# jibanCat/gp_dla_detection

Measured on NVIDIA B200. Metric: qso_spectra_per_sec_10k_dla_samples, higher is better.
Workload: dtype f64

## Files before the change

### gp_dla_detection_b200/csrc/gpdla_i8_kernels.cuh

```cuda
#pragma once
#include "gpdla_kernels.cuh"

namespace gpdla {
namespace i8 {

constexpr int CLUSTER = 4;
constexpr int TS = 32;
constexpr int TM = CLUSTER * TS;
constexpr int WCTAS = 3;
constexpr int NPROD = 8;
constexpr int SPB = TS / NPROD;
constexpr int NCTRL = 4;
constexpr int THREADS = 32 * (NCTRL + NPROD);
constexpr int STAGES = 3;
constexpr double CAP = 0.996;
constexpr int TMEM_COLS = 512;
#ifndef GPDLA_I8P_PROBE
#define GPDLA_I8P_PROBE 0
#endif
constexpr int PROBE = GPDLA_I8P_PROBE;
#ifndef GPDLA_I8P_SHFL_CONV
#define GPDLA_I8P_SHFL_CONV 0
#endif
#ifndef GPDLA_I8P_PF
#define GPDLA_I8P_PF 0
#endif
#ifndef GPDLA_I8P_NCA
#define GPDLA_I8P_NCA 4
#endif
#ifndef GPDLA_I8P_PHASES
#define GPDLA_I8P_PHASES 0
#endif

template <int K, int L>
struct Shape {
  using G = GramShape<K>;
  static constexpr int WBLOCKS = (G::NPAIR <= WCTAS * 80) ? WCTAS : WCTAS + CLUSTER * ((G::NPAIR - WCTAS * 80 + CLUSTER * 80 - 1) / (CLUSTER * 80));
  static constexpr bool EXT = WBLOCKS > WCTAS;
  static constexpr int CPASSES = (WBLOCKS - WCTAS) / CLUSTER;
  static constexpr int NSLOT = WBLOCKS + 1;
  static constexpr int USLOT = WBLOCKS;
  static constexpr int WCOLS = (G::NPAIR + WBLOCKS - 1) / WBLOCKS;
  static constexpr int NW = (WCOLS + 15) / 16 * 16;
  static constexpr int NU = (K + 15) / 16 * 16;
  static constexpr int NMAX = NW > NU ? NW : NU;
  static constexpr int F = 8 * L - 1;
  static constexpr int LBO_A = 128;
  static constexpr int PLANE_A = (KC / 8) * LBO_A;
  static constexpr int SBO_A = PLANE_A * L;
  static constexpr int ROWBLOCK = (TS / 16) * SBO_A;
  static constexpr int A_TILE = (TM / 16) * SBO_A;
  static constexpr int BW_PLANE = NW * KC, BU_PLANE = NU * KC;
  static constexpr int L_BW = L * BW_PLANE;
  static constexpr int B_MAX = L * (BW_PLANE > BU_PLANE ? BW_PLANE : BU_PLANE);
  static constexpr int CHUNK_BYTES = L * (WBLOCKS * BW_PLANE + BU_PLANE);
  static constexpr int B_BUF = B_MAX;
  static constexpr int NCOLTAB = NSLOT * NMAX;
  static constexpr int CSTR = TS + 4;
  static constexpr int NENT = (K + 1) * (K + 2) / 2;
  static_assert(L * NW <= TMEM_COLS && L * NU <= TMEM_COLS, "diagonal accumulators must fit in TMEM");
  static_assert(WBLOCKS * WCOLS >= G::NPAIR && NW <= 80, "column blocks must cover the pair columns");
  static_assert(L >= 2 && L <= 7, "digit count");
  __host__ __device__ static constexpr int b_offset(int slot) { return slot * L * BW_PLANE; }
  __host__ __device__ static constexpr int b_bytes(int slot) { return L * (slot < WBLOCKS ? BW_PLANE : BU_PLANE); }
  __host__ __device__ static constexpr int slot_of_rank(int rank) { return rank < WCTAS ? rank : USLOT; }
  __host__ __device__ static constexpr int gram_column(int slot, int n) {
    return slot < WBLOCKS ? ((n < WCOLS && slot * WCOLS + n < G::NPAIR) ? slot * WCOLS + n : -1) : (n < K ? G::WT * 8 + n : -1);
  }
  __host__ __device__ static constexpr uint64_t digit_bias() {
    uint64_t b = 0;
    for (int i = 0; i < L; ++i) b |= (uint64_t)0x80 << (8 * i);
    return b;
  }
  __host__ __device__ static constexpr double magic() {
    double m = 1.5;
    for (int i = 0; i < 52 - F; ++i) m *= 2.0;
    return m;
  }
  static constexpr size_t OFF_A = 0;
  static constexpr size_t OFF_SX = OFF_A + (size_t)STAGES * A_TILE;
  static constexpr size_t OFF_B = OFF_SX + (size_t)STAGES * ROWBLOCK;
  static constexpr size_t OFF_CS = OFF_B + 2ull * B_BUF;
  static constexpr size_t OFF_RAW = OFF_CS + (EXT ? 0 : (size_t)NENT * CSTR * 8);
  static constexpr size_t OFF_MISC = OFF_RAW + (size_t)TS * RAWS * 8;
};

__constant__ short c_i8_stage[CLUSTER * 128];

struct I8Args {
  double* pix2;
  double* pix8;
  uint8_t* bop;
  double* colscale;
  double* colinv;
  int* status;
  int32_t* f64flag;
  int32_t* f64list;
  uint8_t* adig;
  unsigned long long* phase;
};

__device__ __forceinline__ unsigned long long* phase_ptr(const I8Args& xa) { return GPDLA_I8P_PHASES ? xa.phase : nullptr; }

__device__ __forceinline__ uint32_t cluster_ctarank() { uint32_t r; asm volatile("mov.u32 %0, %%cluster_ctarank;" : "=r"(r)); return r; }
__device__ __forceinline__ void cluster_sync_all() {
  asm volatile("barrier.cluster.arrive.release.aligned;" ::: "memory");
  asm volatile("barrier.cluster.wait.acquire.aligned;" ::: "memory");
}
__device__ __forceinline__ uint32_t mapa(uint32_t saddr, uint32_t rank) {
  uint32_t r;
  asm volatile("mapa.shared::cluster.u32 %0, %1, %2;" : "=r"(r) : "r"(saddr), "r"(rank));
  return r;
}
__device__ __forceinline__ void mbar_wait_d(uint64_t* bar, uint32_t parity, int* status, int code,
                                            unsigned long long* phase = nullptr, unsigned backoff_ns = 0) {
  const uint32_t a = smem_u32(bar);
  const long long t0 = phase ? clock64() : 0;
  for (uint32_t spins = 0;; ++spins) {
    uint32_t ok;
    asm volatile("{\n.reg .pred p;\nmbarrier.try_wait.parity.shared::cta.b64 p, [%1], %2;\nselp.u32 %0, 1, 0, p;\n}\n"
                 : "=r"(ok) : "r"(a), "r"(parity) : "memory");
    if (ok) break;
    if (backoff_ns) __nanosleep(backoff_ns);
    if (spins > 20000000u) {
      if (status) atomicExch(status, code + 100 * (int)(cluster_ctarank() + 1));
      __threadfence_system();
      asm volatile("trap;");
    }
  }
  if (phase) atomicAdd(&phase[8 + code], (unsigned long long)(clock64() - t0));
}
__device__ __forceinline__ void mbar_arrive_expect_tx(uint64_t* bar, uint32_t bytes) { mbar_expect_tx(bar, bytes); }
__device__ __forceinline__ void dsmem_bulk_copy(uint32_t dst_cluster, uint32_t src_cta, uint32_t bytes, uint32_t bar_cluster) {
  asm volatile("cp.async.bulk.shared::cluster.shared::cta.mbarrier::complete_tx::bytes [%0], [%1], %2, [%3];" ::"r"(dst_cluster),
               "r"(src_cta), "r"(bytes), "r"(bar_cluster)
               : "memory");
}
__device__ __forceinline__ void st_cluster_f64(uint32_t addr, double v) {
  asm volatile("st.shared::cluster.f64 [%0], %1;" ::"r"(addr), "d"(v) : "memory");
}
__device__ __forceinline__ uint64_t make_desc(uint32_t saddr, uint32_t lbo, uint32_t sbo) {
  return (uint64_t)((saddr >> 4) & 0x3FFF) | ((uint64_t)((lbo >> 4) & 0x3FFF) << 16) | ((uint64_t)((sbo >> 4) & 0x3FFF) << 32) |
         (1ull << 46);
}
__host__ __device__ constexpr uint32_t make_idesc(int n) {
  return (2u << 4) | (1u << 7) | (1u << 10) | (1u << 15) | ((uint32_t)(n >> 3) << 17) | ((uint32_t)(TM >> 4) << 24);
}
__device__ __forceinline__ void mma_i8(uint32_t tmem_d, uint64_t da, uint64_t db, uint32_t idesc, uint32_t accumulate) {
  asm volatile(
      "{\n.reg .pred p;\nsetp.ne.b32 p, %4, 0;\n"
      "tcgen05.mma.cta_group::1.kind::i8 [%0], %1, %2, %3, {%5, %5, %5, %5}, p;\n}\n" ::"r"(tmem_d),
      "l"(da), "l"(db), "r"(idesc), "r"(accumulate), "r"(0u)
      : "memory");
}
__device__ __forceinline__ void mma_commit(uint64_t* bar) {
  asm volatile("tcgen05.commit.cta_group::1.mbarrier::arrive::one.shared::cluster.b64 [%0];" ::"r"(smem_u32(bar)) : "memory");
}
__device__ __forceinline__ void mma_commit_multicast(uint64_t* bar, uint16_t mask) {
  asm volatile("tcgen05.commit.cta_group::1.mbarrier::arrive::one.shared::cluster.multicast::cluster.b64 [%0], %1;" ::"r"(
                   smem_u32(bar)),
               "h"(mask)
               : "memory");
}

__device__ __forceinline__ void bulk_store_global(void* dst, uint32_t src_cta, uint32_t bytes) {
  asm volatile("cp.async.bulk.global.shared::cta.bulk_group [%0], [%1], %2;" ::"l"(dst), "r"(src_cta), "r"(bytes) : "memory");
}
__device__ __forceinline__ void tma_load_1d_multicast(uint32_t dst_cta, const void* src, uint32_t bytes, uint32_t bar_cta, uint16_t mask) {
  asm volatile("cp.async.bulk.shared::cluster.global.mbarrier::complete_tx::bytes.multicast::cluster [%0], [%1], %2, [%3], %4;" ::"r"(dst_cta),
               "l"(src), "r"(bytes), "r"(bar_cta), "h"(mask)
               : "memory");
}

template <class Sh, int L, int N>
__device__ __forceinline__ void issue_chunk_mmas_fixed(uint32_t tmem_base, uint64_t da0, uint64_t db0, bool accumulate) {
  constexpr int group = 256 / N;
#pragma unroll
  for (int i = L - 1; i >= 0; --i) {
    const uint64_t da = da0 + (uint64_t)((i * Sh::PLANE_A) >> 4);
#pragma unroll
    for (int t0 = 0; t0 <= i; t0 += group) {
      const int nt = (PROBE & 32) ? 1 : ((group < i + 1 - t0) ? group : i + 1 - t0);
      const uint64_t db = db0 + (uint64_t)(((L - 1 - i + t0) * N * KC) >> 4);
      const uint32_t idesc = (PROBE & 16) ? (make_idesc(nt * N) & ~(0x1fu << 24)) | (4u << 24) : make_idesc(nt * N);
      mma_i8(tmem_base + (uint32_t)(t0 * N), da, db, idesc, (accumulate || i < L - 1) ? 1u : 0u);
    }
  }
}

template <int K, int L>
__global__ void __launch_bounds__(NTHREADS) i8_scales_kernel(const QuasarMeta* __restrict__ meta, const double* __restrict__ pix,
                                                             const double* __restrict__ Mq, const double* __restrict__ lam_pad,
                                                             const double* __restrict__ lamh, I8Args xa, int NPIX) {
  using Sh = Shape<K, L>;
  using G = GramShape<K>;
  const int q = blockIdx.x, tid = threadIdx.x;
  const double* pq = pix + (int64_t)q * NPIX * 4;
  double* p2 = xa.pix2 + (int64_t)q * NPIX * 2;
  double2* p8 = reinterpret_cast<double2*>(xa.pix8 + (int64_t)q * NPIX * 8);
  const double* lq = lam_pad + (int64_t)q * (NPIX + 8) + 6;
  const double* lhq = lamh + (int64_t)q * (NPIX + 8) + 6;
  bool unbounded = false;
  for (int i = tid; i < NPIX; i += NTHREADS) {
    const double y = pq[i * 4 + 0], v = pq[i * 4 + 1], mu = pq[i * 4 + 2], om2 = pq[i * 4 + 3];
    const double cw = CAP * (om2 + v);
    const double b = (v >= om2) ? 1.0 / (om2 + v) : 0.5 / sqrt(om2 * v);
    const double yy = fabs(y) + fabs(mu);
    unbounded |= !(v > 0.0) || !isfinite(b) || !isfinite(cw);
    const double cu = (yy > 0.0 && isfinite(b)) ? CAP / (b * yy) : 0.0;
    p2[i * 2 + 0] = cw; p2[i * 2 + 1] = cu;
    p8[i] = make_double2(lq[i], lhq[i]); p8[NPIX + i] = make_double2(y, v);
    p8[2 * NPIX + i] = make_double2(mu, om2); p8[3 * NPIX + i] = make_double2(cw, cu);
  }
  if (__syncthreads_or(unbounded) && tid == 0 && meta[q].nchunks > 0) {
    xa.f64flag[q] = 1;
    xa.f64list[1 + atomicAdd(&xa.f64list[0], 1)] = q;
  }
  const int n_u = meta[q].n_u;
  const double* mq = Mq + (int64_t)q * NPIX * K;
  __shared__ double sM[KC][K + 1];
// ... 213 lines not shown
    asm volatile("tcgen05.alloc.cta_group::1.sync.aligned.shared::cta.b32 [%0], %1;" ::"r"(smem_u32(s_tmem)), "n"(TMEM_COLS));
    asm volatile("tcgen05.relinquish_alloc_permit.cta_group::1.sync.aligned;");
  }
  asm volatile("tcgen05.fence::before_thread_sync;");
  __syncthreads();
  asm volatile("tcgen05.fence::after_thread_sync;");
  const uint32_t tmem_base = *s_tmem;
  cluster_sync_all();

  auto tile_live = [&](int q, const QuasarMeta& m) {
    return m.nchunks > 0 && !(args.active != nullptr && args.active[q] == 0) && xa.f64flag[q] == 0;
  };
  constexpr uint32_t b_bytes = (uint32_t)Sh::L_BW;
  if (warp == 0 && lane == 0) {
    const uint64_t da_stage0 = make_desc(smem_u32(At), Sh::LBO_A, Sh::SBO_A);
    const uint64_t db_buf0 = make_desc(smem_u32(Bt), 128, 256);
    int gc = 0, it = 0;
    for (int t = cluster_id; t < num_tiles; t += num_clusters) {
      const int q = (t % tiles_per_pass) / tiles_per_quasar;
      const QuasarMeta meta = args.meta[q];
      if (!tile_live(q, meta)) continue;
      if (it > 0) mbar_wait_d(bar_tfree, (it - 1) & 1, xa.status, 23, nullptr, 100);
      for (int c = 0; c < meta.nchunks; ++c, ++gc) {
        const int stage = gc % C_STAGES;
        mbar_wait_d(&bar_full[stage], (gc / C_STAGES) & 1, xa.status, 22, nullptr);
        asm volatile("tcgen05.fence::after_thread_sync;");
        const uint64_t da0 = da_stage0 + (uint64_t)(uint32_t)(stage * (Sh::A_TILE >> 4));
        const uint64_t db0 = db_buf0 + (uint64_t)(uint32_t)(stage * (Sh::L_BW >> 4));
        issue_chunk_mmas_fixed<Sh, L, Sh::NW>(tmem_base, da0, db0, c > 0);
        mma_commit_multicast(&bar_empty[stage], (uint16_t)((1u << CLUSTER) - 1));
      }
      mma_commit(bar_acc);
      ++it;
    }
  } else if (warp == 1 && lane == 0) {
    int gc = 0;
    for (int t = cluster_id; t < num_tiles; t += num_clusters) {
      const int pass = t / tiles_per_pass, qt = t % tiles_per_pass;
      const int q = qt / tiles_per_quasar;
      const QuasarMeta meta = args.meta[q];
      if (!tile_live(q, meta)) continue;
      const int slot = WCTAS + CLUSTER * pass + (int)rank;
      const uint8_t* asrc = xa.adig + (int64_t)qt * (args.NPIX / KC) * Sh::A_TILE + rank * Sh::ROWBLOCK;
      const uint8_t* bsrc = xa.bop + (int64_t)q * (args.NPIX / KC) * Sh::CHUNK_BYTES + Sh::b_offset(slot);
      for (int c = 0; c < meta.nchunks; ++c, ++gc) {
        const int stage = gc % C_STAGES;
        mbar_wait_d(&bar_empty[stage], ((gc / C_STAGES) & 1) ^ 1, xa.status, 21, nullptr, 50);
        mbar_expect_tx(&bar_full[stage], (uint32_t)Sh::A_TILE + b_bytes);
        tma_load_1d_multicast(smem_u32(At + stage * Sh::A_TILE) + rank * Sh::ROWBLOCK, asrc + (int64_t)c * Sh::A_TILE, Sh::ROWBLOCK,
                              smem_u32(&bar_full[stage]), (uint16_t)((1u << CLUSTER) - 1));
        tma_load_1d(Bt + stage * Sh::L_BW, bsrc + (int64_t)c * Sh::CHUNK_BYTES, b_bytes, &bar_full[stage]);
      }
    }
  } else if (warp >= 4) {
    const int e = warp & 3, half = (warp - 4) >> 2;
    constexpr int CHALF = (Sh::NW / 2 + 7) / 8 * 8;
    const uint32_t taddr0 = tmem_base + ((uint32_t)(e * 32) << 16);
    int it = 0;
    for (int t = cluster_id; t < num_tiles; t += num_clusters) {
      const int pass = t / tiles_per_pass, qt = t % tiles_per_pass;
      const int q = qt / tiles_per_quasar;
      const QuasarMeta meta = args.meta[q];
      if (!tile_live(q, meta)) continue;
      const int slot = WCTAS + CLUSTER * pass + (int)rank;
      if (lane == 0) mbar_wait_d(bar_acc, it & 1, xa.status, 24, nullptr, 200);
      __syncwarp();
      asm volatile("tcgen05.fence::after_thread_sync;");
      const int64_t row = (int64_t)(qt % tiles_per_quasar) * TM + e * 32 + lane;
      drain_to_gram<Sh, L>(taddr0, Sh::NW, slot, xa.colscale + (int64_t)q * Sh::NCOLTAB + slot * Sh::NMAX,
                           args.gram + ((int64_t)q * args.gram_rows + row) * Sh::G::NCOL, half * CHALF, (half + 1) * CHALF);
      asm volatile("tcgen05.fence::before_thread_sync;");
      __syncwarp();
      if (lane == 0) mbar_arrive(bar_tfree);
      ++it;
    }
  }
  __syncwarp();
  asm volatile("tcgen05.fence::before_thread_sync;");
  cluster_sync_all();
  asm volatile("tcgen05.fence::after_thread_sync;");
  if (warp == 0) asm volatile("tcgen05.dealloc.cta_group::1.sync.aligned.b32 %0, %1;" ::"r"(tmem_base), "n"(TMEM_COLS));
}

template <int K, int L>
struct PShape {
  using Sh = Shape<K, L>;
  static constexpr size_t OFF_MISC = Sh::OFF_MISC;
  __host__ __device__ static constexpr size_t smem_bytes(int num_lines) {
    return OFF_MISC + (size_t)TS * (num_lines + 6) * 8 + 128 * 8 + 4 * TS * 4 + 64 + (size_t)NPROD * 2 * SPB * KC * 8;
  }
};

template <int K, int L, int NL, int MODE>
__global__ void __cluster_dims__(CLUSTER, 1, 1) __launch_bounds__(P_THREADS, 1)
dla_loglik_i8p_kernel(LoglikArgs args, I8Args xa, int num_quasars, int tiles_per_quasar) {
  using Sh = Shape<K, L>;
  constexpr int CSTR = Sh::CSTR;
  const int tid = threadIdx.x, warp = tid >> 5, lane = tid & 31;
  const uint32_t rank = cluster_ctarank();
  const int64_t S = args.S;
  const int cluster_id = blockIdx.x / CLUSTER, num_clusters = gridDim.x / CLUSTER;
  const int num_tiles = num_quasars * tiles_per_quasar;

  extern __shared__ __align__(1024) unsigned char smem_raw[];
  uint8_t* At = smem_raw + Sh::OFF_A;
  uint8_t* Sx = smem_raw + Sh::OFF_SX;
  uint8_t* Bt = smem_raw + Sh::OFF_B;
  double* Cs = reinterpret_cast<double*>(smem_raw + Sh::OFF_CS);
  double* rawbuf = reinterpret_cast<double*>(smem_raw + Sh::OFF_RAW);
  double* s_nhi = reinterpret_cast<double*>(smem_raw + Sh::OFF_MISC);
  double* s_q = s_nhi + TS;
  double* s_ld = s_q + 2 * TS;
  double* s_mult = s_ld + 2 * TS;
  const int num_lines = (NL > 0) ? NL : args.num_lines;
  double* s_K = s_mult + (size_t)TS * num_lines;
  uint64_t* bars = reinterpret_cast<uint64_t*>(s_K + TS);
  uint64_t* bar_full = bars;
  uint64_t* bar_empty = bar_full + STAGES;
  uint64_t* bar_rows = bar_empty + STAGES;
  uint64_t* bar_pfull = bar_rows + STAGES;
  uint64_t* bar_pempty = bar_pfull + 2;
  uint64_t* bar_acc = bar_pempty + 2;
  uint64_t* bar_tfree = bar_acc + 1;
  uint64_t* bar_sq = bar_tfree + 1;
  uint64_t* bar_csfull = bar_sq + 2;
  uint64_t* bar_csfree = bar_csfull + 1;
  uint32_t* s_tmem = reinterpret_cast<uint32_t*>(bars + 32);
  uint64_t* bar_hfull = bars + 64;
  uint64_t* bar_hempty = bar_hfull + 2 * NPROD;
  int* s_part = reinterpret_cast<int*>(bars + 128);
  int* s_so = s_part + 3 * TS;
  double* hbuf = reinterpret_cast<double*>(s_so + TS + 16);

  if (tid == 0) {
    for (int i = 0; i < STAGES; ++i) { mbar_init(&bar_full[i], 1); mbar_init(&bar_empty[i], CLUSTER + (Sh::EXT ? 1 : 0)); mbar_init(&bar_rows[i], NPROD); }
    for (int i = 0; i < 2; ++i) { mbar_init(&bar_pfull[i], 1); mbar_init(&bar_pempty[i], 1); mbar_init(&bar_sq[i], NPROD); }
    mbar_init(bar_acc, 1); mbar_init(bar_tfree, 4); mbar_init(bar_csfull, CLUSTER);
    for (int i = 0; i < 2 * NPROD; ++i) { mbar_init(&bar_hfull[i], 1); mbar_init(&bar_hempty[i], 1); }
    for (int i = 0; i < CLUSTER; ++i) mbar_init(&bar_csfree[i], 4);
    asm volatile("fence.mbarrier_init.release.cluster;" ::: "memory");
  }
  if (warp == 0) {
    asm volatile("tcgen05.alloc.cta_group::1.sync.aligned.shared::cta.b32 [%0], %1;" ::"r"(smem_u32(s_tmem)), "n"(TMEM_COLS));
    asm volatile("tcgen05.relinquish_alloc_permit.cta_group::1.sync.aligned;");
  }
  asm volatile("tcgen05.fence::before_thread_sync;");
  __syncthreads();
  asm volatile("tcgen05.fence::after_thread_sync;");
  const uint32_t tmem_base = *s_tmem;
  cluster_sync_all();

  const int N = rank < WCTAS ? Sh::NW : Sh::NU;
  constexpr int NCA = (MODE == 0) ? GPDLA_I8P_NCA : SPB;
  constexpr bool CONV_B = NCA < SPB;
  constexpr bool SHFL_CONV = GPDLA_I8P_SHFL_CONV && !CONV_B && MODE != 2;
  const int slot = Sh::slot_of_rank((int)rank);
  const uint32_t b_bytes = (uint32_t)Sh::b_bytes(slot);
  auto tile_quasar = [&](int t) { return t / tiles_per_quasar; };
  auto tile_live = [&](int q, const QuasarMeta& m) {
    return m.nchunks > 0 && !(args.active != nullptr && args.active[q] == 0) && xa.f64flag[q] == 0;
  };

  if (warp >= NCTRL + 2 * NPROD) {
    asm volatile("setmaxnreg.inc.sync.aligned.u32 %0;" ::"n"(REG_EPI));
    const int e = warp - NCTRL - 2 * NPROD;
    const uint32_t cs_remote = mapa(smem_u32(Cs), (uint32_t)e) + (uint32_t)lane * 8;
    const uint32_t csfull_remote = mapa(smem_u32(bar_csfull), (uint32_t)e);
    const uint32_t taddr0 = tmem_base + ((uint32_t)(e * 32) << 16);
    int it = 0;
    for (int t = cluster_id; t < num_tiles; t += num_clusters) {
      const int q = tile_quasar(t);
      const QuasarMeta meta = args.meta[q];
      const int64_t s0 = (int64_t)(t % tiles_per_quasar) * TM + (int64_t)rank * TS;
      if (!tile_live(q, meta)) {
        if (lane < 8 && xa.f64flag[q] == 0) {
          const int64_t s = s0 + e * 8 + lane;
          if (s < S) args.sample_log_likelihoods[(int64_t)q * args.sll_stride + s] = NAN;
          else if (s == S && args.log_likelihoods_no_dla) args.log_likelihoods_no_dla[q] = NAN;
        }
        continue;
      }
      if (lane == 0) {
        mbar_wait_d(bar_acc, it & 1, xa.status, 6, phase_ptr(xa), 500);
        if (!Sh::EXT && it > 0) mbar_wait_cluster(&bar_csfree[e], (it - 1) & 1, xa.status, 10, phase_ptr(xa));
      }
      __syncwarp();
      asm volatile("tcgen05.fence::after_thread_sync;");
      const double* cs = xa.colscale + (int64_t)q * Sh::NCOLTAB + slot * Sh::NMAX;
      if constexpr (Sh::EXT) {
        drain_to_gram<Sh, L>(taddr0, N, slot, cs, args.gram + ((int64_t)q * args.gram_rows + (s0 - (int64_t)rank * TS) + e * 32 + lane) * Sh::G::NCOL);
        asm volatile("tcgen05.fence::before_thread_sync;");
        __syncwarp();
        if (lane == 0) mbar_arrive(bar_tfree);
        ++it;
        continue;
      }
      for (int c0 = 0; c0 < ((PROBE & 8) ? 0 : N); c0 += 8) {
        uint32_t v[L][8];
#pragma unroll
        for (int tt = 0; tt < L; ++tt) {
          asm volatile("tcgen05.ld.sync.aligned.32x32b.x8.b32 {%0,%1,%2,%3,%4,%5,%6,%7}, [%8];"
                       : "=r"(v[tt][0]), "=r"(v[tt][1]), "=r"(v[tt][2]), "=r"(v[tt][3]), "=r"(v[tt][4]), "=r"(v[tt][5]),
                         "=r"(v[tt][6]), "=r"(v[tt][7])
                       : "r"(taddr0 + (uint32_t)(tt * N + c0)));
        }
        asm volatile("tcgen05.wait::ld.sync.aligned;" ::: "memory");
#pragma unroll
        for (int jj = 0; jj < 8; ++jj) {
          const int idx = c_i8_stage[rank * 128 + c0 + jj];
          if (idx >= 0) {
            double acc = (double)(int32_t)v[L - 1][jj];
#pragma unroll
            for (int tt = L - 2; tt >= 0; --tt) acc = fma(acc, 256.0, (double)(int32_t)v[tt][jj]);
            st_cluster_f64(cs_remote + (uint32_t)(idx * CSTR * 8), acc * cs[c0 + jj]);
          }
        }
      }
      asm volatile("tcgen05.fence::before_thread_sync;");
      asm volatile("fence.acq_rel.cluster;" ::: "memory");
      __syncwarp();
      if (lane == 0) {
        mbar_arrive(bar_tfree);
        mbar_arrive_cluster(csfull_remote);
        mbar_wait_cluster(bar_csfull, it & 1, xa.status, 11, phase_ptr(xa));
        mbar_wait_d(&bar_sq[it & 1], (it >> 1) & 1, xa.status, 12, phase_ptr(xa), 200);
      }
      __syncwarp();
      if constexpr (!Sh::EXT) {
        if (!(PROBE & 8)) factor_staged<K, CSTR>(Cs, s_q + (it & 1) * TS, s_ld + (it & 1) * TS, e * 8, lane, meta, args, q, s0);
      }
      __syncwarp();
      if (lane == 0) {
        const uint32_t freebar = smem_u32(&bar_csfree[rank]);
        for (uint32_t peer = 0; peer < (uint32_t)CLUSTER; ++peer) mbar_arrive_cluster(mapa(freebar, peer));
      }
      ++it;
    }
  } else if (warp >= NCTRL + NPROD) {
    asm volatile("setmaxnreg.inc.sync.aligned.u32 %0;" ::"n"(REG_B));
    const int pr = warp - NCTRL - NPROD;
    const int row0 = pr * SPB;
    const uint32_t own_block = rank * Sh::ROWBLOCK;
    uint8_t* const wdst0 = (rank < WCTAS) ? At + own_block : Sx;
    uint8_t* const udst0 = (rank < WCTAS) ? Sx : At + own_block;
    const uint32_t wstride = (rank < WCTAS) ? Sh::A_TILE : Sh::ROWBLOCK;
    const uint32_t ustride = (rank < WCTAS) ? Sh::ROWBLOCK : Sh::A_TILE;
    const uint32_t rowoff = (row0 / 16) * Sh::SBO_A + (row0 % 16) + (lane / 8) * Sh::LBO_A + (lane % 8) * 16;
    constexpr uint64_t BIAS = Sh::digit_bias();
    const double MAGIC = Sh::magic();
    const uint64_t KADD = BIAS - (uint64_t)__double_as_longlong(MAGIC);
    const double* hb = hbuf + pr * (2 * SPB * KC) + lane;
    uint64_t* const hfull = bar_hfull + 2 * pr;
    uint64_t* const hempty = bar_hempty + 2 * pr;
    double* myraw = rawbuf + row0 * RAWS;
    int it = 0;
    int stage = 0;
    uint32_t empty_parity = 1;
    uint32_t gh = 0;
    long long w_empty = 0, w_hand = 0;
    for (int t = cluster_id; t < num_tiles; t += num_clusters) {
      const int q = tile_quasar(t);
      const QuasarMeta meta = args.meta[q];
      if (!tile_live(q, meta)) continue;
      const int64_t s0 = (int64_t)(t % tiles_per_quasar) * TM + (int64_t)rank * TS;
      const int nchunks = meta.nchunks;
      const double2* prec = reinterpret_cast<const double2*>(xa.pix8 + (int64_t)q * args.NPIX * 8) + lane;
      const int64_t PL = args.NPIX;
      double qacc[SPB], ldm[SPB];
      int lde[SPB];
#pragma unroll
      for (int ss = 0; ss < SPB; ++ss) { qacc[ss] = 0.0; ldm[ss] = 1.0; lde[ss] = 0; }
      double2 p01n = prec[PL], p23n = prec[2 * PL], p45n = prec[3 * PL];
      if (CONV_B) {
        const uint32_t slot = gh & 1u;
        mbar_wait_d(&hfull[slot], (gh >> 1) & 1u, xa.status, 14);
        if (lane < 6) {
#pragma unroll
          for (int ss = NCA; ss < SPB; ++ss) myraw[ss * RAWS + lane] = hb[(slot * SPB + ss) * KC];
        }
        __syncwarp();
        if (lane == 0) mbar_arrive(&hempty[slot]);
        ++gh;
      }
      for (int c = 0; c < nchunks; ++c) {
        const double y = p01n.x, v = p01n.y, mu = p23n.x, om2 = p23n.y, cw = p45n.x, cu = p45n.y;
        if (c + 1 < nchunks) {
          prec += KC;
          p01n = prec[PL]; p23n = prec[2 * PL]; p45n = prec[3 * PL];
        }
        const uint32_t slot = gh & 1u;
        long long tw0 = GPDLA_I8P_PHASES ? clock64() : 0;
        mbar_wait_d(&hfull[slot], (gh >> 1) & 1u, xa.status, 14);
        if (GPDLA_I8P_PHASES) w_hand += clock64() - tw0;
        double a[SPB];
#pragma unroll
        for (int ss = 0; ss < SPB; ++ss) a[ss] = hb[(slot * SPB + ss) * KC];
        __syncwarp();
        if (lane == 0) mbar_arrive(&hempty[slot]);
        ++gh;
        if (CONV_B) {
#pragma unroll
          for (int ss = NCA; ss < SPB; ++ss) myraw[ss * RAWS + 6 + lane] = a[ss];
          __syncwarp();
          double carry[SPB];
#pragma unroll
          for (int ss = NCA; ss < SPB; ++ss) {
            const double* rb = myraw + ss * RAWS;
            double acc_a = 0.0;
#pragma unroll
            for (int tt = 0; tt < 6; ++tt) acc_a = fma(rb[lane + tt], c_lines.ip[tt], acc_a);
            acc_a = fma(a[ss], c_lines.ip[6], acc_a);
            carry[ss] = rb[KC + (lane < 6 ? lane : 0)];
            a[ss] = (__double2hiint(a[ss]) < 0) ? 1.0 : acc_a;
          }
          __syncwarp();
          if (lane < 6) {
#pragma unroll
            for (int ss = NCA; ss < SPB; ++ss) myraw[ss * RAWS + lane] = carry[ss];
          }
        }
        uint64_t xw[SPB], xu[SPB];
#pragma unroll
        for (int ss = 0; ss < SPB; ++ss) {
          const double a2 = a[ss] * a[ss];
          const double d = fma(a2, om2, v);
          const double rd = fast_rcp(d);
          const double r = fma(-a[ss], mu, y);
          const double t1 = r * rd;
          xw[ss] = ((uint64_t)__double_as_longlong(fma(a2 * rd, cw, MAGIC)) + KADD) ^ BIAS;
          xu[ss] = ((uint64_t)__double_as_longlong(fma(a[ss] * t1, cu, MAGIC)) + KADD) ^ BIAS;
          qacc[ss] = fma(r, t1, qacc[ss]);
          ldm[ss] *= d;
        }
        tw0 = GPDLA_I8P_PHASES ? clock64() : 0;
        mbar_wait_d(&bar_empty[stage], empty_parity, xa.status, 1);
        if (GPDLA_I8P_PHASES) w_empty += clock64() - tw0;
        uint8_t* dW = wdst0 + stage * wstride + rowoff;
        uint8_t* dU = udst0 + stage * ustride + rowoff;
        if (PROBE & 4) {
          uint64_t sink = 0;
#pragma unroll
          for (int ss = 0; ss < SPB; ++ss) sink ^= xw[ss] ^ (xu[ss] << 1);
          if (sink == 0x123456789abcdefull) dW[0] = 1;
        } else {
          store_digit_planes<L, Sh::PLANE_A>(dW, xw);
          store_digit_planes<L, Sh::PLANE_A>(dU, xu);
          asm volatile("fence.proxy.async.shared::cta;" ::: "memory");
        }
        __syncwarp();
        if (lane == 0) mbar_arrive(&bar_rows[stage]);
        if (++stage == STAGES) { stage = 0; empty_parity ^= 1u; }
        if ((c & 7) == 7) {
#pragma unroll
          for (int ss = 0; ss < SPB; ++ss) {
            const int hi = __double2hiint(ldm[ss]);
            const int e2 = ((hi >> 20) & 0x7ff) - 1023;
            lde[ss] += e2;
            ldm[ss] = __hiloint2double(hi - (e2 << 20), __double2loint(ldm[ss]));
          }
        }
      }
#pragma unroll
      for (int ss = 0; ss < SPB; ++ss) {
        const double qs = warp_sum(qacc[ss]);
        const double ld = warp_sum(log(ldm[ss]) + (double)lde[ss] * 0.693147180559945309417);
        if (lane == 0) {
          if (Sh::EXT) {
            double* qd = args.qld + ((int64_t)q * args.gram_rows + s0 + row0 + ss) * 2;
            qd[0] = qs; qd[1] = ld;
          } else {
            s_q[(it & 1) * TS + row0 + ss] = qs; s_ld[(it & 1) * TS + row0 + ss] = ld;
          }
        }
      }
      __syncwarp();
      if (!Sh::EXT && lane == 0) mbar_arrive(&bar_sq[it & 1]);
      if (GPDLA_I8P_PHASES && xa.phase && lane == 0) {
        atomicAdd(&xa.phase[8 + 1], (unsigned long long)w_empty); atomicAdd(&xa.phase[8 + 14], (unsigned long long)w_hand);
        w_empty = w_hand = 0;
        if (pr == 0) atomicAdd(&xa.phase[7], 1ull);
      }
      ++it;
    }
  } else if (warp >= NCTRL) {
    asm volatile("setmaxnreg.inc.sync.aligned.u32 %0;" ::"n"(REG_A));
    const int pr = warp - NCTRL;
    const int row0 = pr * SPB;
    double* myraw = rawbuf + row0 * RAWS;
    double* hb = hbuf + pr * (2 * SPB * KC) + lane;
    uint64_t* const hfull = bar_hfull + 2 * pr;
    uint64_t* const hempty = bar_hempty + 2 * pr;
    uint32_t gh = 0;
    long long w_hand = 0;
    for (int t = cluster_id; t < num_tiles; t += num_clusters) {
      const int q = tile_quasar(t);
      const QuasarMeta meta = args.meta[q];
      if (!tile_live(q, meta)) continue;
      const int64_t s0 = (int64_t)(t % tiles_per_quasar) * TM + (int64_t)rank * TS;
      const int nchunks = meta.nchunks;
      __syncwarp();
      if (lane < SPB) {
        const int i = row0 + lane;
        const int64_t s = s0 + i;
        const bool is_null = s >= S;
        const int64_t so = sample_at(args, is_null ? S - 1 : s);
        const double z = __dadd_rn(meta.min_z_dla, __dmul_rn(meta.max_z_dla - meta.min_z_dla, args.offset_samples[so]));
        s_nhi[i] = is_null ? -1.0 : args.nhi_samples[so];
        s_K[i] = rest_table_offset(args.rt, z, meta.lam_ref);
        s_so[i] = (int)so;
        for (int j = 0; j < num_lines; ++j) s_mult[j * TS + i] = line_multiplier(j, z);
        if (MODE == 2) {
          for (int j = 0; j < args.num_partners; ++j)
            s_part[j * TS + i] = is_null ? 0 : args.partners[((int64_t)q * 3 + j) * S + so];
        }
      }
      __syncwarp();
      const double* lam = args.lam_pad + (int64_t)q * (args.NPIX + 8);
      const double2* pix8 = reinterpret_cast<const double2*>(xa.pix8 + (int64_t)q * args.NPIX * 8);
      double* const cache_q = (MODE != 0) ? args.acache + (int64_t)q * S * args.NPIX : nullptr;

      const double* lamh = args.lamh + (int64_t)q * (args.NPIX + 8);
      double K_mid;
      const int tab_mode = (MODE != 2) ? group_cell<SPB>(args.rt, s_K + row0, K_mid) : 0;
      auto eval_raw = [&](double lambda, double lh, double (&e)[SPB], const RestCell* cell = nullptr) {
        double tau[SPB];
        tau_samples<NL, SPB>(args.rt, tab_mode, K_mid, lambda, lh, s_mult + row0, TS, s_K + row0, num_lines, tau, cell);
        raw_from_tau<SPB, false>(tau, s_nhi + row0, e);
      };
      double eprev[SPB];
      if (MODE != 2) {
        double e[SPB];
        eval_raw(lam[lane < 6 ? lane : 5], lamh[lane < 6 ? lane : 5], e);
        if (CONV_B) {
          const uint32_t slot = gh & 1u;
          mbar_wait_d(&hempty[slot], ((gh >> 1) & 1u) ^ 1u, xa.status, 15);
#pragma unroll
          for (int ss = NCA; ss < SPB; ++ss) hb[(slot * SPB + ss) * KC] = e[ss];
          __syncwarp();
          if (lane == 0) mbar_arrive(&hfull[slot]);
          ++gh;
        }
        if (SHFL_CONV) {
#pragma unroll
          for (int ss = 0; ss < SPB; ++ss) eprev[ss] = __shfl_sync(0xffffffffu, e[ss], (lane + 6) & 31);
        } else if (lane < 6) {
#pragma unroll
          for (int ss = 0; ss < NCA; ++ss) myraw[ss * RAWS + lane] = e[ss];
        }
      }
      double rows_n[4][SPB];
      auto load_rows = [&](int ipix) {
#pragma unroll
        for (int ss = 0; ss < SPB; ++ss) rows_n[0][ss] = cache_q[(int64_t)s_so[row0 + ss] * args.NPIX + ipix];
#pragma unroll
        for (int j = 0; j < 3; ++j)
          if (j < args.num_partners) {
#pragma unroll
            for (int ss = 0; ss < SPB; ++ss) rows_n[1 + j][ss] = cache_q[(int64_t)s_part[j * TS + row0 + ss] * args.NPIX + ipix];
          }
      };
      if (MODE == 2) load_rows(lane);
      const double2* prec = pix8 + lane;
      double2 plln = prec[0];
      double2 plln2 = prec[nchunks > 1 ? KC : 0];
      RestCell cell_n;
      const bool use_cell = GPDLA_I8P_PF && MODE != 2 && tab_mode == 1;
      if (use_cell) rest_table_fetch(args.rt, plln.y, K_mid, cell_n);
      for (int c = 0; c < nchunks; ++c) {
        const int i = c * KC + lane;
        const double lambda = plln.x, lh = plln.y;
        const RestCell cell = cell_n;
        plln = plln2;
        if (c + 2 < nchunks) {
          prec += KC;
          plln2 = prec[KC];
        }
        if (use_cell && c + 1 < nchunks) rest_table_fetch(args.rt, plln.y, K_mid, cell_n);
        double a[SPB];
        if (MODE != 2) {
          double e[SPB];
          eval_raw(lambda, lh, e, use_cell ? &cell : nullptr);
          if (PROBE & 64) {
#pragma unroll
            for (int ss = 0; ss < SPB; ++ss) a[ss] = (__double2hiint(s_nhi[row0 + ss]) < 0) ? 1.0 : e[ss];
          } else {
#pragma unroll
            for (int ss = NCA; ss < SPB; ++ss) a[ss] = (__double2hiint(s_nhi[row0 + ss]) < 0) ? -1.0 : e[ss];
            if (SHFL_CONV) {
#pragma unroll
              for (int ss = 0; ss < SPB; ++ss) {
                double acc_a = 0.0;
#pragma unroll
                for (int tt = 0; tt < 6; ++tt) {
                  const int d = 6 - tt;
                  const double x = (lane >= 32 - d) ? eprev[ss] : e[ss];
                  acc_a = fma(__shfl_sync(0xffffffffu, x, (lane - d) & 31), c_lines.ip[tt], acc_a);
                }
                acc_a = fma(e[ss], c_lines.ip[6], acc_a);
                eprev[ss] = e[ss];
                a[ss] = (__double2hiint(s_nhi[row0 + ss]) < 0) ? 1.0 : acc_a;
              }
            } else if (NCA > 0) {
#pragma unroll
              for (int ss = 0; ss < NCA; ++ss) myraw[ss * RAWS + 6 + lane] = e[ss];
              __syncwarp();
              double carry[SPB];
#pragma unroll
              for (int ss = 0; ss < NCA; ++ss) {
                const double* rb = myraw + ss * RAWS;
                double acc_a = 0.0;
#pragma unroll
                for (int tt = 0; tt < 6; ++tt) acc_a = fma(rb[lane + tt], c_lines.ip[tt], acc_a);
                acc_a = fma(e[ss], c_lines.ip[6], acc_a);
                carry[ss] = rb[KC + (lane < 6 ? lane : 0)];
                a[ss] = (__double2hiint(s_nhi[row0 + ss]) < 0) ? 1.0 : acc_a;
              }
              __syncwarp();
              if (lane < 6) {
#pragma unroll
                for (int ss = 0; ss < NCA; ++ss) myraw[ss * RAWS + lane] = carry[ss];
              }
            }
          }
          if (MODE == 1) {
#pragma unroll
            for (int ss = 0; ss < SPB; ++ss)
              if (s0 + row0 + ss < S) cache_q[(int64_t)s_so[row0 + ss] * args.NPIX + i] = a[ss];
          }
        } else {
#pragma unroll
          for (int ss = 0; ss < SPB; ++ss) a[ss] = rows_n[0][ss];
#pragma unroll
          for (int j = 0; j < 3; ++j)
            if (j < args.num_partners) {
#pragma unroll
              for (int ss = 0; ss < SPB; ++ss) a[ss] = a[ss] * rows_n[1 + j][ss];
            }
          if (c + 1 < nchunks) load_rows(i + KC);
        }
        const uint32_t slot = gh & 1u;
        const long long tw0 = GPDLA_I8P_PHASES ? clock64() : 0;
        mbar_wait_d(&hempty[slot], ((gh >> 1) & 1u) ^ 1u, xa.status, 15);
        if (GPDLA_I8P_PHASES) w_hand += clock64() - tw0;
#pragma unroll
        for (int ss = 0; ss < SPB; ++ss) hb[(slot * SPB + ss) * KC] = a[ss];
        __syncwarp();
        if (lane == 0) mbar_arrive(&hfull[slot]);
        ++gh;
      }
      if (GPDLA_I8P_PHASES && xa.phase && lane == 0) { atomicAdd(&xa.phase[8 + 15], (unsigned long long)w_hand); w_hand = 0; }
    }
  } else {
    asm volatile("setmaxnreg.dec.sync.aligned.u32 %0;" ::"n"(REG_CTRL));
    if (warp == 0 && lane == 0) {
      static_assert(Sh::A_TILE % 16 == 0 && Sh::B_BUF % 16 == 0 && Sh::PLANE_A % 16 == 0, "descriptor offsets are in 16-byte units");
      const uint64_t da_stage0 = make_desc(smem_u32(At), Sh::LBO_A, Sh::SBO_A);
      const uint64_t db_buf0 = make_desc(smem_u32(Bt), 128, 256);
      int gc = 0, it = 0;
      for (int t = cluster_id; t < num_tiles; t += num_clusters) {
        const int q = tile_quasar(t);
        const QuasarMeta meta = args.meta[q];
        if (!tile_live(q, meta)) continue;
        const long long tile_t0 = GPDLA_I8P_PHASES ? clock64() : 0;
        if (it > 0) mbar_wait_d(bar_tfree, (it - 1) & 1, xa.status, 13, phase_ptr(xa), 100);
        for (int c = 0; c < meta.nchunks; ++c, ++gc) {
          const int stage = gc % STAGES, buf = gc & 1;
          mbar_wait_d(&bar_full[stage], (gc / STAGES) & 1, xa.status, 2, phase_ptr(xa), 100);
          mbar_wait_d(&bar_pfull[buf], (gc >> 1) & 1, xa.status, 3, phase_ptr(xa));
          asm volatile("tcgen05.fence::after_thread_sync;");
          const uint64_t da0 = da_stage0 + (uint64_t)(uint32_t)(stage * (Sh::A_TILE >> 4));
          const uint64_t db0 = db_buf0 + (uint64_t)(uint32_t)(buf * (Sh::B_BUF >> 4));
          if (PROBE & 1) { (void)da0; (void)db0; }
          else if (rank < WCTAS) issue_chunk_mmas_fixed<Sh, L, Sh::NW>(tmem_base, da0, db0, c > 0);
          else issue_chunk_mmas_fixed<Sh, L, Sh::NU>(tmem_base, da0, db0, c > 0);
          mma_commit_multicast(&bar_empty[stage], (uint16_t)((1u << CLUSTER) - 1));
          mma_commit(&bar_pempty[buf]);
        }
        mma_commit(bar_acc);
        if (GPDLA_I8P_PHASES && xa.phase) atomicAdd(&xa.phase[6], (unsigned long long)(clock64() - tile_t0));
        ++it;
      }
    } else if (warp == 1 && lane == 0) {
      int gc = 0;
      for (int t = cluster_id; t < num_tiles; t += num_clusters) {
        const int q = tile_quasar(t);
        const QuasarMeta meta = args.meta[q];
        if (!tile_live(q, meta)) continue;
        const uint8_t* bsrc = xa.bop + (int64_t)q * (args.NPIX / KC) * Sh::CHUNK_BYTES + Sh::b_offset(slot);
        for (int c = 0; c < meta.nchunks; ++c, ++gc) {
          const int buf = gc & 1;
          if (gc >= 2) mbar_wait_d(&bar_pempty[buf], ((gc >> 1) - 1) & 1, xa.status, 4, phase_ptr(xa), 100);
          mbar_expect_tx(&bar_pfull[buf], b_bytes);
          tma_load_1d(Bt + buf * Sh::B_BUF, bsrc + (int64_t)c * Sh::CHUNK_BYTES, b_bytes, &bar_pfull[buf]);
        }
      }
    } else if (warp == 2 && lane == 0) {
      int gc = 0;
      for (int t = cluster_id; t < num_tiles; t += num_clusters) {
        const int q = tile_quasar(t);
        const QuasarMeta meta = args.meta[q];
        if (!tile_live(q, meta)) continue;
        for (int c = 0; c < meta.nchunks; ++c, ++gc) {
          const int stage = gc % STAGES;
          mbar_wait_d(&bar_rows[stage], (gc / STAGES) & 1, xa.status, 5, phase_ptr(xa), 100);
          const uint32_t dst_off = smem_u32(At + stage * Sh::A_TILE) + rank * Sh::ROWBLOCK;
          const uint32_t other_rows = smem_u32(Sx + stage * Sh::ROWBLOCK);
          const uint32_t fullbar = smem_u32(&bar_full[stage]);
          if (PROBE & 2) { mbar_arrive(&bar_full[stage]); continue; }
          for (uint32_t peer = 0; peer < (uint32_t)CLUSTER; ++peer) {
            if (peer == rank) continue;
            const uint32_t src = (rank < WCTAS && peer < WCTAS) ? dst_off : other_rows;
            dsmem_bulk_copy(mapa(dst_off, peer), src, Sh::ROWBLOCK, mapa(fullbar, peer));
          }
          mbar_arrive_expect_tx(&bar_full[stage], (CLUSTER - 1) * Sh::ROWBLOCK);
          if constexpr (Sh::EXT) {
            uint8_t* gdst = xa.adig + (((int64_t)q * tiles_per_quasar + (t % tiles_per_quasar)) * (args.NPIX / KC) + c) * Sh::A_TILE +
                            rank * Sh::ROWBLOCK;
            bulk_store_global(gdst, (rank < WCTAS) ? dst_off : other_rows, Sh::ROWBLOCK);
            asm volatile("cp.async.bulk.commit_group;" ::: "memory");
            asm volatile("cp.async.bulk.wait_group.read 0;" ::: "memory");
            mbar_arrive(&bar_empty[stage]);
          }
        }
      }
    }
    __syncwarp();
  }
  asm volatile("tcgen05.fence::before_thread_sync;");
// ... 8 lines not shown
```

Before: 5704.

## Remap stage-B warps to sample-group by pixel-block tiles with shared hand-over slots

Stage-B consumer warps now cover 16 samples by 8 pixels each instead of 4 samples by 32 pixels. Hand-over buffers are shared per group of four warps, with an XOR-swizzled layout and 2 or 3 slots depending on the line count. The per-sample reductions become a cross-warp named-barrier tree plus shuffles. The split-convolution path (NCA) is removed, so the producers always do the full convolution. The goal is bank-conflict-free digit stores into the MMA tile, checked by constexpr asserts. The cost is extra named-barrier syncs in the reduction and coupling between warps through group-level mbarriers.

```diff
diff --git a/gp_dla_detection_b200/csrc/gpdla_i8_kernels.cuh b/gp_dla_detection_b200/csrc/gpdla_i8_kernels.cuh
--- a/gp_dla_detection_b200/csrc/gpdla_i8_kernels.cuh
+++ b/gp_dla_detection_b200/csrc/gpdla_i8_kernels.cuh
@@ -24,9 +24,6 @@
 #endif
 #ifndef GPDLA_I8P_PF
 #define GPDLA_I8P_PF 0
-#endif
-#ifndef GPDLA_I8P_NCA
-#define GPDLA_I8P_NCA 4
 #endif
 #ifndef GPDLA_I8P_PHASES
 #define GPDLA_I8P_PHASES 0
@@ -136,6 +133,10 @@
                "r"(src_cta), "r"(bytes), "r"(bar_cluster)
                : "memory");
 }
+template <int ID, int THREADS>
+__device__ __forceinline__ void named_barrier_sync() {
+  asm volatile("bar.sync %0, %1;" ::"n"(ID), "n"(THREADS) : "memory");
+}
 __device__ __forceinline__ void st_cluster_f64(uint32_t addr, double v) {
   asm volatile("st.shared::cluster.f64 [%0], %1;" ::"r"(addr), "d"(v) : "memory");
 }
@@ -515,12 +516,114 @@
   if (warp == 0) asm volatile("tcgen05.dealloc.cta_group::1.sync.aligned.b32 %0, %1;" ::"r"(tmem_base), "n"(TMEM_COLS));
 }
 
+struct StageB {
+  static constexpr int GROUPS = TS / 16;
+  static constexpr int WARPS = NPROD / GROUPS;
+  static constexpr int HAND_SLOT = 16 * KC;
+  __host__ __device__ static constexpr int hand_slots(int num_lines) { return num_lines <= 3 ? 3 : 2; }
+  static constexpr int RED = GROUPS * 2 * SPB * 32;
+  __host__ __device__ static constexpr int group(int pr) { return pr / WARPS; }
+  __host__ __device__ static constexpr int pblock(int pr) { return pr % WARPS; }
+  __host__ __device__ static constexpr int sample(int pr, int lane, int ss) { return 16 * group(pr) + SPB * (lane & 3) + ss; }
+  __host__ __device__ static constexpr int pixel(int pr, int lane) { return 8 * pblock(pr) + (lane >> 2); }
+  __host__ __device__ static constexpr int hand(int sl, int pix) { return sl * KC + (pix ^ (8 * ((sl / SPB) & 1))); }
+  template <class Sh>
+  __host__ __device__ static constexpr int tile_byte(int sample, int pix) {
+    return (sample / 16) * Sh::SBO_A + (pix / 8) * Sh::LBO_A + (pix % 8) * 16 + sample % 16;
+  }
+};
+
+__host__ __device__ constexpr int bank_wavefronts(const int (&addr)[32], int bytes) {
+  int words[32][64] = {}, n[32] = {}, worst = 0;
+  for (int l = 0; l < 32; ++l)
+    for (int w = addr[l] / 4; w < (addr[l] + bytes) / 4; ++w) {
+      bool seen = false;
+      for (int i = 0; i < n[w % 32]; ++i) seen |= words[w % 32][i] == w;
+      if (!seen) words[w % 32][n[w % 32]++] = w;
+      worst = n[w % 32] > worst ? n[w % 32] : worst;
+    }
+  return worst;
+}
+template <class Sh>
+__host__ __device__ constexpr bool stage_b_stores_conflict_free() {
+  for (int pr = 0; pr < NPROD; ++pr) {
+    int addr[32] = {};
+    for (int l = 0; l < 32; ++l) {
+      addr[l] = StageB::tile_byte<Sh>(StageB::sample(pr, l, 0), StageB::pixel(pr, l));
+      if (addr[l] % 4 != 0) return false;
+    }
+    if (bank_wavefronts(addr, 4) != 1) return false;
+  }
+  return Sh::PLANE_A % 128 == 0 && Sh::SBO_A % 128 == 0;
+}
+__host__ __device__ constexpr int hand_over_wavefronts(bool b_read) {
+  int worst = 0;
+  for (int pr = 0; pr < NPROD; ++pr)
+    for (int ss = 0; ss < SPB; ++ss) {
+      int addr[32] = {};
+      for (int l = 0; l < 32; ++l)
+        addr[l] = 8 * (b_read ? StageB::hand(StageB::sample(pr, l, ss) % 16, StageB::pixel(pr, l)) : StageB::hand((pr * SPB + ss) % 16, l));
+      const int w = bank_wavefronts(addr, 8);
+      worst = w > worst ? w : worst;
+    }
+  return worst;
+}
+__host__ __device__ constexpr bool stage_b_tiles_block() {
+  unsigned cover[TS] = {};
+  for (int pr = 0; pr < NPROD; ++pr)
+    for (int l = 0; l < 32; ++l)
+      for (int ss = 0; ss < SPB; ++ss) {
+        const int s = StageB::sample(pr, l, ss), p = StageB::pixel(pr, l);
+        if (s < 0 || s >= TS || p < 0 || p >= KC || ((cover[s] >> p) & 1u)) return false;
+        cover[s] |= 1u << p;
+        if (StageB::group(pr) != s / 16 || StageB::hand(s % 16, p) != StageB::hand(s % 16 - ss, p) + ss * KC) return false;
+      }
+  for (int s = 0; s < TS; ++s)
+    if (cover[s] != 0xffffffffu) return false;
+  return true;
+}
+static_assert(KC == 32 && TS == 32 && SPB == 4 && StageB::WARPS * 8 == KC, "stage-B mapping: 2 groups x 4 pixel blocks of 8");
+static_assert(stage_b_tiles_block(), "stage-B warps must tile the chunk's (sample, pixel) block exactly");
+static_assert(hand_over_wavefronts(true) == 2 && hand_over_wavefronts(false) == 2, "hand-over accesses: 2 wavefronts per 256 bytes");
+
+__device__ __forceinline__ void group_sum(double (&v)[SPB], double* red, int g, int pb) {
+  auto sync = [g] {
+    if (g == 0) named_barrier_sync<1, 32 * StageB::WARPS>();
+    else named_barrier_sync<2, 32 * StageB::WARPS>();
+  };
+  static_assert(StageB::GROUPS == 2, "one named barrier per group");
+  if (pb >= 2) {
+#pragma unroll
+    for (int ss = 0; ss < SPB; ++ss) red[((pb & 1) * SPB + ss) * 32] = v[ss];
+  }
+  sync();
+  if (pb < 2) {
+#pragma unroll
+    for (int ss = 0; ss < SPB; ++ss) v[ss] += red[((pb & 1) * SPB + ss) * 32];
+  }
+  if (pb == 1) {
+#pragma unroll
+    for (int ss = 0; ss < SPB; ++ss) red[(SPB + ss) * 32] = v[ss];
+  }
+  sync();
+  if (pb == 0) {
+#pragma unroll
+    for (int ss = 0; ss < SPB; ++ss) {
+      v[ss] += red[(SPB + ss) * 32];
+#pragma unroll
+      for (int o = 16; o >= 4; o >>= 1) v[ss] += __shfl_xor_sync(0xffffffffu, v[ss], o);
+    }
+  }
+  sync();
+}
+
 template <int K, int L>
 struct PShape {
   using Sh = Shape<K, L>;
   static constexpr size_t OFF_MISC = Sh::OFF_MISC;
   __host__ __device__ static constexpr size_t smem_bytes(int num_lines) {
-    return OFF_MISC + (size_t)TS * (num_lines + 6) * 8 + 128 * 8 + 4 * TS * 4 + 64 + (size_t)NPROD * 2 * SPB * KC * 8;
+    return OFF_MISC + (size_t)TS * (num_lines + 6) * 8 + 128 * 8 + 4 * TS * 4 + 64 + (size_t)StageB::GROUPS * StageB::hand_slots(num_lines) * StageB::HAND_SLOT * 8 +
+           (size_t)StageB::RED * 8;
   }
 };
 
@@ -559,17 +662,23 @@
   uint64_t* bar_csfull = bar_sq + 2;
   uint64_t* bar_csfree = bar_csfull + 1;
   uint32_t* s_tmem = reinterpret_cast<uint32_t*>(bars + 32);
+  constexpr int HS = (NL > 0) ? StageB::hand_slots(NL) : 2;
   uint64_t* bar_hfull = bars + 64;
-  uint64_t* bar_hempty = bar_hfull + 2 * NPROD;
+  uint64_t* bar_hempty = bar_hfull + HS * StageB::GROUPS;
   int* s_part = reinterpret_cast<int*>(bars + 128);
   int* s_so = s_part + 3 * TS;
   double* hbuf = reinterpret_cast<double*>(s_so + TS + 16);
+  double* s_red = hbuf + StageB::GROUPS * HS * StageB::HAND_SLOT;
+  static_assert(stage_b_stores_conflict_free<Sh>(), "stage-B digit stores must be one wavefront each");
+  static_assert(PShape<K, L>::smem_bytes(MAX_LINES) <= 227 * 1024 && PShape<K, L>::smem_bytes(3) <= 227 * 1024,
+                "shared memory beyond the opt-in limit");
+  static_assert(2 * HS * StageB::GROUPS <= 64, "hand-over barriers must fit their 64 slots");
 
   if (tid == 0) {
     for (int i = 0; i < STAGES; ++i) { mbar_init(&bar_full[i], 1); mbar_init(&bar_empty[i], CLUSTER + (Sh::EXT ? 1 : 0)); mbar_init(&bar_rows[i], NPROD); }
     for (int i = 0; i < 2; ++i) { mbar_init(&bar_pfull[i], 1); mbar_init(&bar_pempty[i], 1); mbar_init(&bar_sq[i], NPROD); }
     mbar_init(bar_acc, 1); mbar_init(bar_tfree, 4); mbar_init(bar_csfull, CLUSTER);
-    for (int i = 0; i < 2 * NPROD; ++i) { mbar_init(&bar_hfull[i], 1); mbar_init(&bar_hempty[i], 1); }
+    for (int i = 0; i < HS * StageB::GROUPS; ++i) { mbar_init(&bar_hfull[i], StageB::WARPS); mbar_init(&bar_hempty[i], StageB::WARPS); }
     for (int i = 0; i < CLUSTER; ++i) mbar_init(&bar_csfree[i], 4);
     asm volatile("fence.mbarrier_init.release.cluster;" ::: "memory");
   }
@@ -584,9 +693,7 @@
   cluster_sync_all();
 
   const int N = rank < WCTAS ? Sh::NW : Sh::NU;
-  constexpr int NCA = (MODE == 0) ? GPDLA_I8P_NCA : SPB;
-  constexpr bool CONV_B = NCA < SPB;
-  constexpr bool SHFL_CONV = GPDLA_I8P_SHFL_CONV && !CONV_B && MODE != 2;
+  constexpr bool SHFL_CONV = GPDLA_I8P_SHFL_CONV && MODE != 2;
   const int slot = Sh::slot_of_rank((int)rank);
   const uint32_t b_bytes = (uint32_t)Sh::b_bytes(slot);
   auto tile_quasar = [&](int t) { return t / tiles_per_quasar; };
@@ -672,20 +779,20 @@
   } else if (warp >= NCTRL + NPROD) {
     asm volatile("setmaxnreg.inc.sync.aligned.u32 %0;" ::"n"(REG_B));
     const int pr = warp - NCTRL - NPROD;
-    const int row0 = pr * SPB;
+    const int g = StageB::group(pr), pb = StageB::pblock(pr);
+    const int pix = StageB::pixel(pr, lane);
     const uint32_t own_block = rank * Sh::ROWBLOCK;
-    uint8_t* const wdst0 = (rank < WCTAS) ? At + own_block : Sx;
-    uint8_t* const udst0 = (rank < WCTAS) ? Sx : At + own_block;
+    const uint32_t rowoff = StageB::tile_byte<Sh>(StageB::sample(pr, lane, 0), pix);
+    uint8_t* const wdst0 = ((rank < WCTAS) ? At + own_block : Sx) + rowoff;
+    uint8_t* const udst0 = ((rank < WCTAS) ? Sx : At + own_block) + rowoff;
     const uint32_t wstride = (rank < WCTAS) ? Sh::A_TILE : Sh::ROWBLOCK;
     const uint32_t ustride = (rank < WCTAS) ? Sh::ROWBLOCK : Sh::A_TILE;
-    const uint32_t rowoff = (row0 / 16) * Sh::SBO_A + (row0 % 16) + (lane / 8) * Sh::LBO_A + (lane % 8) * 16;
     constexpr uint64_t BIAS = Sh::digit_bias();
     const double MAGIC = Sh::magic();
     const uint64_t KADD = BIAS - (uint64_t)__double_as_longlong(MAGIC);
-    const double* hb = hbuf + pr * (2 * SPB * KC) + lane;
-    uint64_t* const hfull = bar_hfull + 2 * pr;
-    uint64_t* const hempty = bar_hempty + 2 * pr;
-    double* myraw = rawbuf + row0 * RAWS;
+    const double* hb = hbuf + g * (HS * StageB::HAND_SLOT) + StageB::hand(StageB::sample(pr, lane, 0) % 16, pix);
+    uint64_t* const hfull = bar_hfull + HS * g;
+    uint64_t* const hempty = bar_hempty + HS * g;
     int it = 0;
     int stage = 0;
     uint32_t empty_parity = 1;
@@ -697,61 +804,29 @@
       if (!tile_live(q, meta)) continue;
       const int64_t s0 = (int64_t)(t % tiles_per_quasar) * TM + (int64_t)rank * TS;
       const int nchunks = meta.nchunks;
-      const double2* prec = reinterpret_cast<const double2*>(xa.pix8 + (int64_t)q * args.NPIX * 8) + lane;
+      const double2* prec = reinterpret_cast<const double2*>(xa.pix8 + (int64_t)q * args.NPIX * 8) + pix;
       const int64_t PL = args.NPIX;
       double qacc[SPB], ldm[SPB];
       int lde[SPB];
 #pragma unroll
       for (int ss = 0; ss < SPB; ++ss) { qacc[ss] = 0.0; ldm[ss] = 1.0; lde[ss] = 0; }
       double2 p01n = prec[PL], p23n = prec[2 * PL], p45n = prec[3 * PL];
-      if (CONV_B) {
-        const uint32_t slot = gh & 1u;
-        mbar_wait_d(&hfull[slot], (gh >> 1) & 1u, xa.status, 14);
-        if (lane < 6) {
-#pragma unroll
-          for (int ss = NCA; ss < SPB; ++ss) myraw[ss * RAWS + lane] = hb[(slot * SPB + ss) * KC];
-        }
-        __syncwarp();
-        if (lane == 0) mbar_arrive(&hempty[slot]);
-        ++gh;
-      }
       for (int c = 0; c < nchunks; ++c) {
         const double y = p01n.x, v = p01n.y, mu = p23n.x, om2 = p23n.y, cw = p45n.x, cu = p45n.y;
         if (c + 1 < nchunks) {
           prec += KC;
           p01n = prec[PL]; p23n = prec[2 * PL]; p45n = prec[3 * PL];
         }
-        const uint32_t slot = gh & 1u;
+        const uint32_t slot = gh % HS;
         long long tw0 = GPDLA_I8P_PHASES ? clock64() : 0;
-        mbar_wait_d(&hfull[slot], (gh >> 1) & 1u, xa.status, 14);
+        mbar_wait_d(&hfull[slot], (gh / HS) & 1u, xa.status, 14);
         if (GPDLA_I8P_PHASES) w_hand += clock64() - tw0;
         double a[SPB];
 #pragma unroll
-        for (int ss = 0; ss < SPB; ++ss) a[ss] = hb[(slot * SPB + ss) * KC];
+        for (int ss = 0; ss < SPB; ++ss) a[ss] = hb[slot * StageB::HAND_SLOT + ss * KC];
         __syncwarp();
         if (lane == 0) mbar_arrive(&hempty[slot]);
         ++gh;
-        if (CONV_B) {
-#pragma unroll
-          for (int ss = NCA; ss < SPB; ++ss) myraw[ss * RAWS + 6 + lane] = a[ss];
-          __syncwarp();
-          double carry[SPB];
-#pragma unroll
-          for (int ss = NCA; ss < SPB; ++ss) {
-            const double* rb = myraw + ss * RAWS;
-            double acc_a = 0.0;
-#pragma unroll
-            for (int tt = 0; tt < 6; ++tt) acc_a = fma(rb[lane + tt], c_lines.ip[tt], acc_a);
-            acc_a = fma(a[ss], c_lines.ip[6], acc_a);
-            carry[ss] = rb[KC + (lane < 6 ? lane : 0)];
-            a[ss] = (__double2hiint(a[ss]) < 0) ? 1.0 : acc_a;
-          }
-          __syncwarp();
-          if (lane < 6) {
-#pragma unroll
-            for (int ss = NCA; ss < SPB; ++ss) myraw[ss * RAWS + lane] = carry[ss];
-          }
-        }
         uint64_t xw[SPB], xu[SPB];
 #pragma unroll
         for (int ss = 0; ss < SPB; ++ss) {
@@ -768,8 +843,8 @@
         tw0 = GPDLA_I8P_PHASES ? clock64() : 0;
         mbar_wait_d(&bar_empty[stage], empty_parity, xa.status, 1);
         if (GPDLA_I8P_PHASES) w_empty += clock64() - tw0;
-        uint8_t* dW = wdst0 + stage * wstride + rowoff;
-        uint8_t* dU = udst0 + stage * ustride + rowoff;
+        uint8_t* dW = wdst0 + stage * wstride;
+        uint8_t* dU = udst0 + stage * ustride;
         if (PROBE & 4) {
           uint64_t sink = 0;
 #pragma unroll
@@ -793,16 +868,20 @@
           }
         }
       }
-#pragma unroll
-      for (int ss = 0; ss < SPB; ++ss) {
-        const double qs = warp_sum(qacc[ss]);
-        const double ld = warp_sum(log(ldm[ss]) + (double)lde[ss] * 0.693147180559945309417);
-        if (lane == 0) {
+      double* const red = s_red + g * (2 * SPB * 32) + lane;
+      group_sum(qacc, red, g, pb);
+#pragma unroll
+      for (int ss = 0; ss < SPB; ++ss) ldm[ss] = log(ldm[ss]) + (double)lde[ss] * 0.693147180559945309417;
+      group_sum(ldm, red, g, pb);
+      if (pb == 0 && lane < 4) {
+        const int row0 = 16 * g + SPB * lane;
+#pragma unroll
+        for (int ss = 0; ss < SPB; ++ss) {
           if (Sh::EXT) {
             double* qd = args.qld + ((int64_t)q * args.gram_rows + s0 + row0 + ss) * 2;
-            qd[0] = qs; qd[1] = ld;
+            qd[0] = qacc[ss]; qd[1] = ldm[ss];
           } else {
-            s_q[(it & 1) * TS + row0 + ss] = qs; s_ld[(it & 1) * TS + row0 + ss] = ld;
+            s_q[(it & 1) * TS + row0 + ss] = qacc[ss]; s_ld[(it & 1) * TS + row0 + ss] = ldm[ss];
           }
         }
       }
@@ -820,9 +899,10 @@
     const int pr = warp - NCTRL;
     const int row0 = pr * SPB;
     double* myraw = rawbuf + row0 * RAWS;
-    double* hb = hbuf + pr * (2 * SPB * KC) + lane;
-    uint64_t* const hfull = bar_hfull + 2 * pr;
-    uint64_t* const hempty = bar_hempty + 2 * pr;
+    const int g = StageB::group(pr);
+    double* hb = hbuf + g * (HS * StageB::HAND_SLOT) + StageB::hand(row0 % 16, lane);
+    uint64_t* const hfull = bar_hfull + HS * g;
+    uint64_t* const hempty = bar_hempty + HS * g;
     uint32_t gh = 0;
     long long w_hand = 0;
     for (int t = cluster_id; t < num_tiles; t += num_clusters) {
@@ -864,21 +944,12 @@
       if (MODE != 2) {
         double e[SPB];
         eval_raw(lam[lane < 6 ? lane : 5], lamh[lane < 6 ? lane : 5], e);
-        if (CONV_B) {
-          const uint32_t slot = gh & 1u;
-          mbar_wait_d(&hempty[slot], ((gh >> 1) & 1u) ^ 1u, xa.status, 15);
-#pragma unroll
-          for (int ss = NCA; ss < SPB; ++ss) hb[(slot * SPB + ss) * KC] = e[ss];
-          __syncwarp();
-          if (lane == 0) mbar_arrive(&hfull[slot]);
-          ++gh;
-        }
         if (SHFL_CONV) {
 #pragma unroll
           for (int ss = 0; ss < SPB; ++ss) eprev[ss] = __shfl_sync(0xffffffffu, e[ss], (lane + 6) & 31);
         } else if (lane < 6) {
 #pragma unroll
-          for (int ss = 0; ss < NCA; ++ss) myraw[ss * RAWS + lane] = e[ss];
+          for (int ss = 0; ss < SPB; ++ss) myraw[ss * RAWS + lane] = e[ss];
         }
       }
       double rows_n[4][SPB];
@@ -917,8 +988,6 @@
 #pragma unroll
             for (int ss = 0; ss < SPB; ++ss) a[ss] = (__double2hiint(s_nhi[row0 + ss]) < 0) ? 1.0 : e[ss];
           } else {
-#pragma unroll
-            for (int ss = NCA; ss < SPB; ++ss) a[ss] = (__double2hiint(s_nhi[row0 + ss]) < 0) ? -1.0 : e[ss];
             if (SHFL_CONV) {
 #pragma unroll
               for (int ss = 0; ss < SPB; ++ss) {
@@ -933,13 +1002,13 @@
                 eprev[ss] = e[ss];
                 a[ss] = (__double2hiint(s_nhi[row0 + ss]) < 0) ? 1.0 : acc_a;
               }
-            } else if (NCA > 0) {
-#pragma unroll
-              for (int ss = 0; ss < NCA; ++ss) myraw[ss * RAWS + 6 + lane] = e[ss];
+            } else {
+#pragma unroll
+              for (int ss = 0; ss < SPB; ++ss) myraw[ss * RAWS + 6 + lane] = e[ss];
               __syncwarp();
               double carry[SPB];
 #pragma unroll
-              for (int ss = 0; ss < NCA; ++ss) {
+              for (int ss = 0; ss < SPB; ++ss) {
                 const double* rb = myraw + ss * RAWS;
                 double acc_a = 0.0;
 #pragma unroll
@@ -951,7 +1020,7 @@
               __syncwarp();
               if (lane < 6) {
 #pragma unroll
-                for (int ss = 0; ss < NCA; ++ss) myraw[ss * RAWS + lane] = carry[ss];
+                for (int ss = 0; ss < SPB; ++ss) myraw[ss * RAWS + lane] = carry[ss];
               }
             }
           }
@@ -971,12 +1040,12 @@
             }
           if (c + 1 < nchunks) load_rows(i + KC);
         }
-        const uint32_t slot = gh & 1u;
+        const uint32_t slot = gh % HS;
         const long long tw0 = GPDLA_I8P_PHASES ? clock64() : 0;
-        mbar_wait_d(&hempty[slot], ((gh >> 1) & 1u) ^ 1u, xa.status, 15);
+        mbar_wait_d(&hempty[slot], ((gh / HS) & 1u) ^ 1u, xa.status, 15);
         if (GPDLA_I8P_PHASES) w_hand += clock64() - tw0;
 #pragma unroll
-        for (int ss = 0; ss < SPB; ++ss) hb[(slot * SPB + ss) * KC] = a[ss];
+        for (int ss = 0; ss < SPB; ++ss) hb[slot * StageB::HAND_SLOT + ss * KC] = a[ss];
         __syncwarp();
         if (lane == 0) mbar_arrive(&hfull[slot]);
         ++gh;
```

Result: no change. 5757, median of 6 (+0.9%).
